# yzGuu830/efficient-speech-codec

Measured on AMD Instinct MI355X. Metric: audio-seconds/sec encode+decode, ESC-Base 9kbps 3s@16kHz, higher is better.
Workload: dtype f32 (fp32 storage and accumulation everywhere; the K = C contractions of the MLPs, of the attention's Q / K / V projections, of PatchMerge / PatchSplit and of the de-embedding run on the fp16 matrix cores with every fp32 operand split into two fp16 terms under power-of-two scales (range-safe by cons

## Files before the change

efficient-speech-codec_amd/csrc/escx_api.cpp:

```cpp
#include <hip/hip_runtime.h>

#include <algorithm>
#include <cmath>
#include <cstdlib>
#include <cstring>
#include <map>
#include <mutex>
#include <tuple>
#include <utility>
#include <vector>

#include "escx_internal.h"
#include "launchers.h"

using namespace escx;

static void part_layout(escx_handle_s* h, int B, int T, int* k, int* per, int* pass) {
    *k = std::min(n_parts(h, B), h->n_sets);
    *pass = std::max(1, std::min(pass_clips(h, B, T), h->sets[0].shp.B));
    *per = *k <= 1 ? B : (B + *k - 1) / *k;
}

template <class F>
static int run_halves(escx_handle_s* h, int B, int T, hipStream_t st, F part) {
// ... 179 lines not shown
             ln_rows(2, cur, h->xn, L.sub_g, L.sub_b, map, H2 * W, tokens, B * H2 * W, L.C, L.Cp, st));
        PROF("merge_gemm", 2.0 * B * H2 * W * 2 * L.C * L.Cout, (double)B * H2 * W * (2 * L.C + L.Cout) * 4,
             gemm_store(h->xn, 2 * L.Cp, B * H2 * W, L.sub_w, L.CoutP, 2 * L.Cp, y, L.CoutP, nullptr, st));
        }
        *Hout = H2;
    } else if (L.scale == 2) {
        int src2 = -1;
        if (h->use_fused)
            PROF("split_fused" + (h->prof ? "[C=" + std::to_string(L.C) + "]" : std::string()), 2.0 * M * L.C * 2 * L.Cout, (double)M * (L.C + 2 * L.Cout) * 4,
                 src2 = rowgemm_fused(1, cur, y, L.sub_g, L.sub_b, L.sub_wf, nullptr, M, tokens, tokens, L.C, L.Cp, 2 * L.CoutP, 1, H, W, L.CoutP, st, L.sub_x3, x3_nt(h)));
        if (src2 != 0) {
        PROF("split_ln", 0, 2.0 * M * L.C * 4,
             ln_rows(0, cur, h->xn, L.sub_g, L.sub_b, nullptr, tokens, tokens, M, L.C, L.Cp, st));
        PROF("split_gemm", 2.0 * M * L.C * 2 * L.Cout, (double)M * (L.C + 2 * L.Cout) * 4,
             gemm_split(h->xn, L.Cp, M, L.sub_w, 2 * L.CoutP, L.Cp, y, H, W, L.CoutP, st));
        }
        *Hout = 2 * H;
    } else {
        *Hout = H;
    }
    return launch_ok(L.prefix.c_str());
}

static int run_stft(escx_handle_s* h, const float* wave, int B, int L, int T, float* spec, hipStream_t st) {
    PROF("stft_dft_gemm", 2.0 * B * T * h->cfg.win_length * 2 * h->F, ((double)B * L + (double)B * T * 2 * h->F) * 4,
         gemm_frames(wave, B, L, T, h->cfg.hop_length, h->left - h->n_fft / 2, h->dft_w, h->cfg.in_dim * h->Fp, h->winP, spec, st));
    return launch_ok("stft");
}

static int run_patch_embed(escx_handle_s* h, const float* spec, int B, int T, int W, float* tok, hipStream_t st) {
    const escx_config& c = h->cfg;
    const int H0 = c.in_freq / c.patch_f;
    const double toks = (double)B * H0 * W;
    PROF("patch_embed_gemm", 2.0 * toks * c.in_dim * c.patch_f * c.patch_t * h->C0, ((double)B * T * 2 * h->F + toks * h->C0) * 4,
         gemm_patch(spec, B, T, c.in_dim, h->Fp, H0, W, c.patch_f, c.patch_t, h->pe_w, h->C0p, h->Kpe, tok, h->pe_b, st));
    PROF("patch_embed_ln", 0, 2 * toks * h->C0 * 4,
         ln_rows(0, tok, tok, h->pe_g, h->pe_beta, nullptr, H0 * W, H0 * W, B * H0 * W, h->C0, h->C0p, st));
    return launch_ok("patch_embed");
}

static int run_encoder(escx_handle_s* h, const Shapes& s, hipStream_t st) {
    int rc, H = s.H0, Hn;
    if ((rc = run_patch_embed(h, h->spec, s.B, s.T, s.W, h->stageA, st))) return rc;
    if ((rc = run_layer(h, h->layers[0], h->stageA, h->enc_hs[0], s.B, H, s.W, &Hn, st))) return rc;
    for (int i = 0; i + 1 < h->n; ++i) {
        if ((rc = run_layer(h, h->layers[1 + i], h->enc_hs[i], h->enc_hs[i + 1], s.B, H, s.W, &Hn, st))) return rc;
        H = Hn;
    }
    return 0;
}

static int ensure_pvq_tables(escx_handle_s* h, hipStream_t st) {
    if (!h->pvq_tab_stale) return 0;
    const escx_config& c = h->cfg;
    const int G = c.group_size, Ksz = c.codebook_size;
    const bool on = h->pvq_table;
    auto grab = [&](void** buf, size_t bytes) -> bool { return *buf || hipMalloc(buf, bytes) == hipSuccess; };
    if (on && !h->iota_codes) {
        std::vector<long long> iota((size_t)G * Ksz);
        for (int g = 0; g < G; ++g) for (int k = 0; k < Ksz; ++k) iota[(size_t)g * Ksz + k] = k;
        ESCX_HIP(hipMalloc((void**)&h->iota_codes, iota.size() * sizeof(long long)));
        ESCX_HIP(hipMemcpy(h->iota_codes, iota.data(), iota.size() * sizeof(long long), hipMemcpyHostToDevice));
    }
    for (Quant& q : h->quants) {
        if (!on || !q.tab_ok) { if (q.tab) { ESCX_HIP(hipDeviceSynchronize()); (void)hipFree(q.tab); q.tab = nullptr; } continue; }
        if (!q.tab) ESCX_HIP(hipMalloc((void**)&q.tab, (size_t)Ksz * q.Kq * sizeof(float)));
// ... 53 lines not shown
    const int Tq = W / c.overlap, M = B * Tq;
    const int splits = pvq_down_splits(M, q.Kq, q.Cp);
    if ((size_t)splits * M * q.Nz > h->zpart_cap) ESCX_FAIL(ESCX_ERR_STATE, "split-K scratch too small");
    const double vec = (double)c.overlap * q.Hq * q.C;
    PROF("pvq_down_gemm", 2.0 * M * vec * q.d, (double)M * vec * (dec ? 2 : 1) * 4,
         gemm_pvq_down(enc, dec, B, q.Hq, W, q.Cp, c.overlap, q.wd, q.Nz, q.Kq, h->zpart, splits, st));
    int src_rc = 0;
    PROF("pvq_search", 2.0 * M * c.group_size * c.codebook_size * q.d, ((double)c.group_size * c.codebook_size * q.d + (double)M * c.group_size * q.d) * 4,
         src_rc = pvq_search(h->zpart, splits, M, q.Nz, q.cbn, q.c2, q.cbraw, c.group_size, c.codebook_size, q.d, q.dt, Tq, codes, bstride,
                             loss, 1.0f / ((float)Tq * q.d * c.group_size), c.l2norm, st));
    if (src_rc) ESCX_FAIL(ESCX_ERR_UNSUPPORTED, "codebook_dim %d unsupported by the search kernel", q.d);
    return launch_ok("pvq_encode");
}

static int run_pvq_decode(escx_handle_s* h, const Quant& q, const long long* codes, long long bstride, const float* dec, int B, int W,
                          float* out, hipStream_t st) {
    const escx_config& c = h->cfg;
    const double vec = (double)c.overlap * q.Hq * q.C, Mv = (double)B * (W / c.overlap);
    const bool special = h->pvq_up_kernel;
    if (q.tab && special) {
        PROF("pvq_tab_add", 0, Mv * vec * (dec ? 3 : 2) * 4,
             pvq_tab_add(codes, bstride, q.tab, q.gq, c.group_size, c.codebook_size, B, q.Hq, W, q.Cp, c.overlap, dec, out, st));
        return launch_ok("pvq_decode");
    }
    int urc = -1;
    if (special)
        PROF("pvq_up_gemm", 2.0 * Mv * vec * q.d, Mv * vec * (dec ? 2 : 1) * 4,
             urc = pvq_up(codes, bstride, q.cbraw, c.group_size, c.codebook_size, q.dt, B, q.Hq, W, q.Cp, c.overlap, q.wup, q.Kq, q.Kup, dec, out, st));
    if (urc != 0) {
        if (special && h->prof && !h->prof_recs.empty()) h->prof_recs.pop_back();
    PROF("pvq_up_gemm", 2.0 * Mv * vec * q.d, Mv * vec * (dec ? 2 : 1) * 4,
         gemm_pvq_up(codes, bstride, q.cbraw, c.group_size, c.codebook_size, q.dt, B, q.Hq, W, q.Cp, c.overlap, q.wup, q.Kq, q.Kup, dec, out, st));
    }
    return launch_ok("pvq_decode");
}

static int run_pvq_quantize(escx_handle_s* h, const Quant& q, const float* enc, const float* dec, int B, int W, long long* codes, long long bstride,
                            float* loss, float* out, hipStream_t st) {
    const escx_config& c = h->cfg;
    if (h->pvq_fused) {
        const int Tq = W / c.overlap, M = B * Tq;
        const double vec = (double)c.overlap * q.Hq * q.C;
        int frc = -1;
        PROF(out ? "pvq_fused" : "pvq_fused_codes", 2.0 * M * vec * q.d * (out ? 2 : 1) + 2.0 * M * c.group_size * c.codebook_size * q.d,
             (double)M * vec * ((dec ? 2 : 1) + (out ? (dec ? 2 : 1) : 0)) * 4,
             frc = pvq_fused(enc, dec, B, q.Hq, W, q.Cp, c.overlap, q.wdf, q.Nz, q.Kq, pvq_down_splits(M, q.Kq, q.Cp), pvq_down_bk(q.Cp), q.cbn, q.c2, q.cbraw,
                             c.group_size, c.codebook_size, q.d, q.dt, q.wup, q.tab, q.gq, out, codes, bstride, loss, 1.0f / ((float)Tq * q.d * c.group_size), c.l2norm, st));
        if (frc == 0) return launch_ok("pvq_quantize");
        if (h->prof && !h->prof_recs.empty()) h->prof_recs.pop_back();
    }
    int rc;
    if ((rc = run_pvq_encode(h, q, enc, dec, B, W, codes, bstride, loss, st))) return rc;
    if (out && (rc = run_pvq_decode(h, q, codes, bstride, dec, B, W, out, st))) return rc;
    return 0;
}

static int run_deembed(escx_handle_s* h, const float* tok, int B, int W, float* rspec, hipStream_t st) {
    const escx_config& c = h->cfg;
    const int H0 = c.in_freq / c.patch_f;
    if (!h->deembed_two_stage && c.in_dim * h->Q <= 16) {
        const double tk = (double)B * H0 * W;
        int hrc = -1;
        if (h->deembed_halo)
            PROF("deembed_composed7x7", 2.0 * tk * 49 * h->C0 * c.in_dim * h->Q, (tk * h->C0 + tk * c.in_dim * h->Q) * 4,
                 hrc = deembed7_fused(tok, B, H0, W, h->C0p, h->dch_w, h->dcc_b, rspec, c.patch_f, c.patch_t, c.in_dim, h->Fp, st, h->dch_x2));
        if (hrc != 0)
// ... 52 lines not shown
        if ((rc = run_layer(h, h->layers[n + i], dec, other, s.B, H, s.W, &Hn, st))) return rc;
        std::swap(dec, other); H = Hn;
    }
    return 0;
}

extern "C" int escx_encode(escx_handle h, const float* wave, int B, int L, int S, int64_t* codes, int* fh, int* fw, void* stream) {
    if (h && h->kind == 1) return rvq_encode(h, wave, B, L, nullptr, S, codes, fh, fw, stream);
    int rc = check_ready(h); if (rc) return rc;
    if (!wave || !codes) ESCX_FAIL(ESCX_ERR_INVALID_ARG, "null pointer");
    if (S < 1 || S > h->cfg.max_streams) ESCX_FAIL(ESCX_ERR_INVALID_ARG, "num_streams=%d outside [1, %d]", S, h->cfg.max_streams);
    if (L <= h->n_fft / 2) ESCX_FAIL(ESCX_ERR_INVALID_ARG, "n_samples=%d too short for reflect padding of %d", L, h->n_fft / 2);
    Shapes s; if ((rc = ensure_ws(h, B, frames_of(h, L), &s))) return rc;
    const long long cstride = (long long)S * h->cfg.group_size * s.Tq;
    if ((rc = ensure_pvq_tables(h, (hipStream_t)stream))) return rc;
    rc = run_halves(h, B, s.T, (hipStream_t)stream, [&](int b0, int nb, hipStream_t st) -> int {
        Shapes sp = s; sp.B = nb; int r;
        if ((r = run_stft(h, wave + (size_t)b0 * L, nb, L, sp.T, h->spec, st))) return r;
        if ((r = run_encoder(h, sp, st))) return r;
        return run_csvq_encode(h, sp, S, (long long*)codes + b0 * cstride, st);
    });
    if (rc) return rc;
    if (fh) *fh = s.encH[h->n - 1];
    if (fw) *fw = s.W;
    return ESCX_OK;
}

static int run_csvq_decode(escx_handle_s* h, const long long* codes, int B, int S, int Hb, int W, float* rspec, hipStream_t st) {
    const escx_config& c = h->cfg;
    const int n = h->n, G = c.group_size, Tq = W / c.overlap;
    const long long bstride = (long long)S * G * Tq, sstride = (long long)G * Tq;
    int rc, H = Hb, Hn;
    float* dec = h->decA; float* other = h->decB;
    if ((rc = run_pvq_decode(h, h->quants[0], codes, bstride, nullptr, B, W, dec, st))) return rc;
    for (int i = 0; i + 1 < n; ++i) {
        if (i < S - 1 && (rc = run_pvq_decode(h, h->quants[i + 1], codes + (i + 1) * sstride, bstride, dec, B, W, dec, st))) return rc;
        if ((rc = run_layer(h, h->layers[n + i], dec, other, B, H, W, &Hn, st))) return rc;
        std::swap(dec, other); H = Hn;
    }
    if ((rc = run_layer(h, h->layers[2 * n - 1], dec, other, B, H, W, &Hn, st))) return rc;
    return run_deembed(h, other, B, W, rspec, st);
}

extern "C" int escx_decode(escx_handle h, const int64_t* codes, int B, int S, int fh, int fw, float* wave_out, float* recon_feat,
                           void* stream) {
    if (h && h->kind == 1) return rvq_decode(h, codes, B, S, nullptr, fh, fw, wave_out, recon_feat, stream);
    int rc = check_infer_ready(h); if (rc) return rc;
    if (!codes || !wave_out) ESCX_FAIL(ESCX_ERR_INVALID_ARG, "null pointer");
    const escx_config& c = h->cfg;
    if (S < 1 || S > c.max_streams) ESCX_FAIL(ESCX_ERR_INVALID_ARG, "codes.size(1)=%d outside [1, %d]", S, c.max_streams);
    if (fw < 1 || fw % c.overlap) ESCX_FAIL(ESCX_ERR_ASSERT, "Time dimension must be multiple of overlap");
    Shapes s; if ((rc = ensure_ws(h, B, frames_for_width(h, fw), &s))) return rc;
    if (s.W != fw || s.encH[h->n - 1] != fh) ESCX_FAIL(ESCX_ERR_INVALID_ARG, "feat_shape (%d,%d) does not match the model (%d,%d)", fh, fw, s.encH[h->n - 1], s.W);
    const int T2 = c.patch_t * fw, out_len = c.hop_length * (T2 - 1);
    const long long cstride = (long long)S * c.group_size * (fw / c.overlap);
    if ((rc = ensure_pvq_tables(h, (hipStream_t)stream))) return rc;
    rc = run_halves(h, B, s.T, (hipStream_t)stream, [&](int b0, int nb, hipStream_t st) -> int {
        int r;
        if ((r = run_csvq_decode(h, (const long long*)codes + b0 * cstride, nb, S, fh, fw, h->rspec, st))) return r;
        if ((r = run_istft(h, h->rspec, nb, T2, wave_out + (size_t)b0 * out_len, st))) return r;
        if (recon_feat) spec_unpad(h, h->rspec, recon_feat + (size_t)b0 * T2 * c.in_dim * h->F, (long long)nb * T2, st);
        return launch_ok("decode");
    });
    return rc;
}

static int forward_impl(escx_handle h, const float* wave, const float* feat, int B, int L, int T, int S, int64_t* codes, float* wave_out,
                        float* raw_feat, float* recon_feat, float* cm_loss, void* stream) {
    if (h && h->kind == 1) return rvq_forward(h, wave, feat, B, wave ? L : T, nullptr, S, codes, wave_out, raw_feat, recon_feat, cm_loss, stream);
// ... 119 lines not shown
    return 0;
}

static int upload_plan(escx_handle_s* h, const MixPlan& p, int32_t* dev, hipStream_t st) {
    ESCX_HIP(hipMemcpyAsync(dev, p.ints.data(), p.ints.size() * sizeof(int32_t), hipMemcpyHostToDevice, st));
    return 0;
}

static int clips_over(const int* S, int B, int j) { int c = 0; while (c < B && S[c] > j) ++c; return c; }

static int run_csvq_encode_streams(escx_handle_s* h, const Shapes& s, const int* S, long long* codes, long long bstride, hipStream_t st) {
    const int n = h->n;
    const long long sstride = (long long)h->cfg.group_size * s.Tq;
    int rc, H = s.encH[n - 1], Hn;
    float* dec = h->decA; float* other = h->decB;
    int nref = clips_over(S, s.B, 1);
    if ((rc = run_pvq_quantize(h, h->quants[0], h->enc_hs[n - 1], nullptr, s.B, s.W, codes, bstride, nullptr, nref ? dec : nullptr, st))) return rc;
    for (int i = 0; nref > 0; ++i) {
        const int nq = nref;
        nref = clips_over(S, nq, i + 2);
        if ((rc = run_pvq_quantize(h, h->quants[i + 1], h->enc_hs[n - 1 - i], dec, nq, s.W, codes + (i + 1) * sstride, bstride, nullptr, nref ? dec : nullptr, st))) return rc;
        if (!nref) break;
        if ((rc = run_layer(h, h->layers[n + i], dec, other, nref, H, s.W, &Hn, st))) return rc;
        std::swap(dec, other); H = Hn;
    }
    return 0;
}

static int run_csvq_decode_streams(escx_handle_s* h, const long long* codes, long long bstride, int B, const int* S, int Hb, int W, float* rspec, hipStream_t st) {
    const int n = h->n;
    const long long sstride = (long long)h->cfg.group_size * (W / h->cfg.overlap);
    int rc, H = Hb, Hn;
    float* dec = h->decA; float* other = h->decB;
    if ((rc = run_pvq_decode(h, h->quants[0], codes, bstride, nullptr, B, W, dec, st))) return rc;
    for (int i = 0; i + 1 < n; ++i) {
        const int nq = clips_over(S, B, i + 1);
        if (nq && (rc = run_pvq_decode(h, h->quants[i + 1], codes + (i + 1) * sstride, bstride, dec, nq, W, dec, st))) return rc;
        if ((rc = run_layer(h, h->layers[n + i], dec, other, B, H, W, &Hn, st))) return rc;
        std::swap(dec, other); H = Hn;
    }
    if ((rc = run_layer(h, h->layers[2 * n - 1], dec, other, B, H, W, &Hn, st))) return rc;
    return run_deembed(h, other, B, W, rspec, st);
}

extern "C" int escx_encode_streams(escx_handle h, const float* wave, int B, int L, const int32_t* streams, int64_t* codes, int* fh, int* fw,
                                   void* stream) {
    if (h && h->kind == 1) return rvq_encode(h, wave, B, L, streams, 0, codes, fh, fw, stream);
    int rc = check_ready(h); if (rc) return rc;
    if (!wave || !codes) ESCX_FAIL(ESCX_ERR_INVALID_ARG, "null pointer");
    int Smax = 0; if ((rc = check_streams(h, B, streams, &Smax))) return rc;
    if (L <= h->n_fft / 2) ESCX_FAIL(ESCX_ERR_INVALID_ARG, "n_samples=%d too short for reflect padding of %d", L, h->n_fft / 2);
    Shapes s; if ((rc = ensure_ws(h, B, frames_of(h, L), &s))) return rc;
    MixPlan p; plan_streams(h, B, s.T, streams, Smax, &p);
    const int GT = h->cfg.group_size * s.Tq;
    const long long cstride = (long long)Smax * GT;
    int32_t* maps; float* wave_ws; long long* codes_ws;
    MixBufs mb; mb.add(&maps, p.ints.size()); mb.add(&wave_ws, (size_t)B * L); mb.add(&codes_ws, (size_t)B * cstride);
    if ((rc = mix_alloc(h, mb))) return rc;
    hipStream_t st = (hipStream_t)stream;
    if ((rc = ensure_pvq_tables(h, st))) return rc;
    if ((rc = upload_plan(h, p, maps, st))) return rc;
    PROF("mix_gather", 0, 2.0 * B * L * 4, rows_permute(wave, wave_ws, maps, B, L, st));
    rc = run_halves(h, B, s.T, st, [&](int b0, int nb, hipStream_t sti) -> int {
        Shapes sp = s; sp.B = nb; int r;
        if ((r = run_stft(h, wave_ws + (size_t)b0 * L, nb, L, sp.T, h->spec, sti))) return r;
        if ((r = run_encoder(h, sp, sti))) return r;
        return run_csvq_encode_streams(h, sp, p.S_ws() + b0, codes_ws + b0 * cstride, cstride, sti);
    });
    if (rc) return rc;
// ... 450 lines not shown
```

efficient-speech-codec_amd/csrc/escx_internal.h:

```cpp
#pragma once
#include <hip/hip_runtime.h>
#include <cstdarg>
#include <cstdint>
#include <cstdio>
#include <map>
#include <string>
#include <tuple>
#include <vector>

#include "../../include/escx.h"

namespace escx {

inline int rup(int x, int m) { return (x + m - 1) / m * m; }

void set_error(const char* fmt, ...);

#define ESCX_FAIL(code, ...) do { ::escx::set_error(__VA_ARGS__); return (code); } while (0)
#define ESCX_HIP(expr) do { hipError_t _e = (expr); if (_e != hipSuccess) { \
        ::escx::set_error("%s failed: %s (%s:%d)", #expr, hipGetErrorString(_e), __FILE__, __LINE__); return ESCX_ERR_HIP; } } while (0)

struct Param { std::vector<float> data; std::vector<int64_t> shape; };

struct Arena {
// ... 66 lines not shown
namespace escx {
int make_shapes(escx_handle_s* h, int B, int T, Shapes* out);
int check_infer_ready(escx_handle_s* h);
void free_train_state(escx_handle_s* h);
int get_map(escx_handle_s* h, int H, int W, int shift, const int** out);
int check_ready(escx_handle_s* h);
float* stream_scratch(hipStream_t st, int slot, size_t floats);
int launch_ok(const char* what);
int build_gather_map(escx_handle_s* h);
void use_set(escx_handle_s* h, int i);
int n_parts(escx_handle_s* h, int B);
int ensure_ws(escx_handle_s* h, int B, int T, Shapes* s, int min_set_clips = 0);
int pass_clips(escx_handle_s* h, int B, int T);
}

struct escx_handle_s : escx::WsFields {
    escx_config cfg;
    int kind = 0;
    int num_rvqs = 0;
    int device = 0;
    int n = 0;
    int F = 0, Fp = 0, n_fft = 0, left = 0, winP = 0, Kpe = 0, C0 = 0, C0p = 0, Q = 0;
    std::map<std::string, escx::Param> params;
    std::vector<std::string> required;
    bool finalized = false;
    bool use_fused = true;
    bool use_fused_attn = true;
    int prec = 2;
    int mlp_x3_max = 384, attn_x3_max = 384;
    bool rowgemm_x3 = true, pvq_table = true;
    int attn_gs_tokens = 600;
    bool mlp_split_fold = true;
    bool pvq_fused = true, pvq_up_kernel = true;
    bool prof_serial = false;
    int ws = 4;

    escx::Arena wts;
    std::vector<escx::Layer> layers;
    std::vector<escx::Quant> quants;
    float *pe_w = nullptr, *pe_b = nullptr, *pe_g = nullptr, *pe_beta = nullptr;
    float *dc1_w = nullptr, *dc1_b = nullptr, *dc2_w = nullptr, *dc2_b = nullptr;
    float *dft_w = nullptr, *idft_w = nullptr, *win2 = nullptr;
    float *dcc_w = nullptr, *dcc_b = nullptr, *dcv_w = nullptr, *dcv_b = nullptr;
    float* dch_w = nullptr;
    void* dch_x2 = nullptr;
    void* dch_x2_buf = nullptr;
    float *dc1_wT = nullptr, *idft_wT = nullptr;
    float* dft_wT = nullptr;

    std::vector<std::string> flat_keys;
    std::vector<size_t> flat_off, flat_numel;
    size_t flat_total = 0;
    int* gmap = nullptr;
    float* garena = nullptr;
    std::vector<std::pair<size_t, size_t>> grad_regions;
    long long* grad_seg = nullptr; int grad_nseg = 0; long long grad_seg_total = 0;
    escx::Arena tape;
    void* train_state = nullptr;
    bool train_x3_stale = true;
    bool pvq_tab_stale = true;
    long long* iota_codes = nullptr;
    bool composed_stale = false;
    bool deembed_halo = true;
    bool deembed_two_stage = false;

    static constexpr int MAX_PARTS = 4;
// ... 43 lines not shown
```

efficient-speech-codec_amd/csrc/escx_params.cpp:

```cpp
#include <hip/hip_runtime.h>

#include <algorithm>
#include <cmath>
#include <cstdlib>
#include <cstring>
#include <map>
#include <mutex>
#include <tuple>

#include "escx_internal.h"
#include "launchers.h"

using namespace escx;

namespace escx {
static thread_local std::string g_err;
void set_error(const char* fmt, ...) {
    char buf[1024];
    va_list ap; va_start(ap, fmt); vsnprintf(buf, sizeof(buf), fmt, ap); va_end(ap);
    g_err = buf;
}
}

extern "C" const char* escx_last_error(void) { return g_err.c_str(); }
// ... 101 lines not shown
            K.push_back(p + "up_projs." + std::to_string(g) + ".weight");
        }
    for (const char* k : {"proj.weight", "proj.bias", "norm.weight", "norm.bias"}) K.push_back(std::string("encoder.patch_embed.") + k);
    for (const Layer& L : h->layers) {
        for (int j = 0; j < c.swin_depth; ++j) add_block_keys(K, L.prefix + "swint_blocks." + std::to_string(j) + ".");
        if (L.scale) {
            K.push_back(L.prefix + "subsample.norm.weight"); K.push_back(L.prefix + "subsample.norm.bias");
            K.push_back(L.prefix + (L.scale == 1 ? "subsample.down.weight" : "subsample.up.weight"));
        }
    }
    for (const char* k : {"de_proj1.weight", "de_proj1.bias", "de_proj2.weight", "de_proj2.bias"})
        K.push_back(std::string("decoder.patch_deembed.") + k);
    return 0;
}

static int env_defaults(escx_handle_s* h) {
    auto flag = [](const char* name, bool dflt) { const char* e = getenv(name); return (e && e[0]) ? e[0] == '1' : dflt; };
    auto off = [](const char* name) { const char* e = getenv(name); return e && e[0] == '0'; };
    auto num = [](const char* name, int dflt) { const char* e = getenv(name); return (e && e[0]) ? atoi(e) : dflt; };
    h->use_fused = !flag("ESCX_NO_FUSED", false);
    h->use_fused_attn = !flag("ESCX_NO_FUSED_ATTN", false);
    h->deembed_two_stage = flag("ESCX_DEEMBED_TWO_STAGE", false);
    h->deembed_halo = !flag("ESCX_DEEMBED_GEMM", false);
    if (getenv("ESCX_STREAMS") && getenv("ESCX_STREAMS")[0]) { h->parts = std::min(std::max(num("ESCX_STREAMS", 2), 1), (int)escx_handle_s::MAX_PARTS); h->parts_forced = true; }
    h->chunk_frames = num("ESCX_CHUNK_FRAMES", h->chunk_frames);
    h->mlp_x3_max = num("ESCX_MLP_X3", h->mlp_x3_max);
    h->attn_x3_max = num("ESCX_ATTN_X3", h->attn_x3_max);
    h->rowgemm_x3 = !off("ESCX_ROWGEMM_X3");
    h->pvq_table = !off("ESCX_PVQ_TABLE");
    h->attn_gs_tokens = num("ESCX_ATTN_GS_TOKENS", h->attn_gs_tokens);
    h->mlp_split_fold = !off("ESCX_MLP_SPLIT_FOLD");
    h->pvq_fused = !off("ESCX_PVQ_FUSED");
    h->pvq_up_kernel = !off("ESCX_PVQ_UP_KERNEL");
    h->prof_serial = flag("ESCX_PROF_SERIAL", false);
    if (num("ESCX_X3_TERMS", 2) == 3) h->prec = 3;
    if (const char* e = getenv("ESCX_PRECISION")) {
        if (e[0]) {
            const std::string v(e);
            if (v == "fp32" || v == "0") h->prec = 0; else if (v == "bf16x3" || v == "3") h->prec = 3; else if (v == "f16x2" || v == "2") h->prec = 2;
            else ESCX_FAIL(ESCX_ERR_INVALID_ARG, "ESCX_PRECISION=%s (fp32 | bf16x3 | f16x2)", e);
        }
    }
    return 0;
}

static int create_impl(const escx_config* cfg, int kind, int num_rvqs, int device, escx_handle* out) {
    int ndev = 0;
    ESCX_HIP(hipGetDeviceCount(&ndev));
    if (device < 0 || device >= ndev) ESCX_FAIL(ESCX_ERR_INVALID_ARG, "device %d out of range (%d visible)", device, ndev);
    escx_handle_s* h = new escx_handle_s();
    h->cfg = *cfg; h->device = device;
    h->kind = kind; h->num_rvqs = num_rvqs;
    int erc = env_defaults(h);
    if (erc) { delete h; return erc; }
    int rc = build_geometry(h);
    if (rc) { delete h; return rc; }
    *out = h;
    return ESCX_OK;
}

extern "C" int escx_create(const escx_config* cfg, int device, escx_handle* out) {
    if (!cfg || !out) ESCX_FAIL(ESCX_ERR_INVALID_ARG, "null argument");
    return create_impl(cfg, 0, 0, device, out);
}

extern "C" int escx_create_rvq(const escx_rvq_config* cfg, int device, escx_handle* out) {
// ... 744 lines not shown
```

efficient-speech-codec_amd/csrc/fused_pvq.h:

```cpp
#pragma once
#include <hip/hip_runtime.h>
#include "gemm_engine.h"
#include "kernels.h"

namespace escx {

struct PvqFusedArgs {
    const float* enc; const float* dec;
    const float* wd;
    const float* cbn; const float* c2; const float* cbraw;
    const float* wup;
    const float* tab; const float* gq;
    float* out;
    long long* codes; long long bstride;
    float* loss; float loss_scale;
    int M, Tq, Hq, Wd, Cp, ov, Kq, k_per_z, splits;
    int G, Ksz, d, l2norm;
    unsigned long long* trace;
};

constexpr int PVQF_WAVES = 16;
constexpr int PVQF_GMAX = 4;
template <int NT> constexpr int pvqf_lds_floats() { return PVQF_WAVES * 16 * (16 * NT + 4); }

// ... 249 lines not shown
                    for (int r = 0; r < 4; ++r) acc = __builtin_amdgcn_mfma_f32_16x16x4f32(wf[u][c][r], zf[c][r], acc, 0, 0, 0);
                if constexpr (DEC) acc += dv[u];
                if (live && nt0 + u < NTo) st4(a.out + idx[u], acc);
            }
        }
    }
    PVQ_TS(5)
#undef PVQ_TS
}

struct PvqTabAddArgs {
    const long long* codes; long long bstride; const float* tab; const float* gq; const float* dec; float* out;
    int G, Ksz, Tq, Hq, Wd, Cp, ov; long long n4;
};
__global__ __launch_bounds__(256) void pvq_tab_add_kernel(PvqTabAddArgs a) {
    ESCX_SET_PRIO_SMALL();
    const long long i = (long long)blockIdx.x * 256 + threadIdx.x;
    if (i >= a.n4) return;
    const int c4 = a.Cp >> 2;
    const long long row = i / c4; const int c = (int)(i - row * c4) * 4;
    const int w = (int)(row % a.Wd); const long long bh = row / a.Wd; const int h = (int)(bh % a.Hq); const int b = (int)(bh / a.Hq);
    const int t = w / a.ov, o = w - t * a.ov;
    const int g = (int)a.gq[(((o * a.Hq + h) * a.Cp) + c) >> 2];
    f32x4 v = zero4();
    if (g >= 0) {
        long long code = a.codes[(size_t)b * a.bstride + (size_t)g * a.Tq + t];
        code = code < 0 ? 0 : (code >= a.Ksz ? a.Ksz - 1 : code);
        v = ld4(a.tab + ((size_t)h * a.ov * a.Ksz + (size_t)a.ov * code + o) * a.Cp + c);
    }
    if (a.dec) v += ld4(a.dec + i * 4);
    st4(a.out + i * 4, v);
}

}
```

efficient-speech-codec_amd/csrc/gemm_engine.h:

```cpp
#pragma once
#include <hip/hip_runtime.h>
#include <cstdlib>
#include <type_traits>

#include "launch_prof.h"

#ifdef ESCX_SMALL_PRIO
#define ESCX_SET_PRIO_SMALL() __builtin_amdgcn_s_setprio(ESCX_SMALL_PRIO)
#else
#define ESCX_SET_PRIO_SMALL()
#endif

namespace escx {

typedef float f32x4 __attribute__((ext_vector_type(4)));

__device__ __forceinline__ f32x4 ld4(const float* p) { return *reinterpret_cast<const f32x4*>(p); }
__device__ __forceinline__ void st4(float* p, f32x4 v) { *reinterpret_cast<f32x4*>(p) = v; }
__device__ __forceinline__ f32x4 zero4() { f32x4 z = {0.f, 0.f, 0.f, 0.f}; return z; }

template <class E, class = void> struct epi_is_rowwise : std::false_type {};
template <class E> struct epi_is_rowwise<E, std::enable_if_t<E::ROWWISE>> : std::true_type {};

template <int BM, int BN, int BK, class Loader, class Epi>
// ... 270 lines not shown
    r = fmaf(r, u, -4.556713975034654e-05f);
    r = fmaf(r, u, 0.0005925663863308728f);
    r = fmaf(r, u, -0.004739245865494013f);
    r = fmaf(r, u, 0.026361873373389244f);
    r = fmaf(r, u, -0.10997311770915985f);
    r = fmaf(r, u, -0.6319426894187927f);
    r = fmaf(r, u, -1.130163311958313f);
    r = fmaf(r, u, 0.00030238047474995255f);
    const float b = copysignf(1.0f - exp_fast(r), x);
    return t <= 0.92f ? a : b;
}
__device__ __forceinline__ float gelu_bf(float x) {
    const float a = fabsf(x);
    float r = -1.6904631365832756e-06f;
    r = fmaf(r, a, 2.5084045773837715e-05f);
    r = fmaf(r, a, -0.0001144662601291202f);
    r = fmaf(r, a, -0.0003233331080991775f);
    r = fmaf(r, a, 0.007333371322602034f);
    r = fmaf(r, a, -0.052714187651872635f);
    r = fmaf(r, a, -0.4591154456138611f);
    r = fmaf(r, a, -1.151123285293579f);
    r = fmaf(r, a, 1.126017423302983e-06f - 1.0f);
    return fmaf(-fabsf(x), __builtin_amdgcn_exp2f(r), fmaxf(x, 0.0f));
}

struct EpiStore {
    float* out; int ldo; const float* bias;
    __device__ __forceinline__ void store(int m, int n, f32x4 v, int) const {
        if (bias) v += ld4(bias + n);
        st4(out + (size_t)m * ldo + n, v);
    }
};

struct EpiGelu {
    float* out; int ldo; const float* bias;
    __device__ __forceinline__ void store(int m, int n, f32x4 v, int) const {
        v += ld4(bias + n);
        v[0] = gelu_erf(v[0]); v[1] = gelu_erf(v[1]); v[2] = gelu_erf(v[2]); v[3] = gelu_erf(v[3]);
        st4(out + (size_t)m * ldo + n, v);
    }
};

struct EpiResidual {
    float* out; int ldo; const float* bias; const float* res;
    __device__ __forceinline__ void store(int m, int n, f32x4 v, int) const {
        v += ld4(bias + n);
        st4(out + (size_t)m * ldo + n, ld4(res + (size_t)m * ldo + n) + v);
    }
};

struct EpiQkv {
    float* out; int ldo; const float* bias; int nq; float scale;
    __device__ __forceinline__ void store(int m, int n, f32x4 v, int) const {
        v += ld4(bias + n);
        if (n < nq) v *= scale;
        st4(out + (size_t)m * ldo + n, v);
    }
};

struct EpiProjScatter {
    float* out; const float* shortcut; const float* bias; const int* map; int slots, tokens, Cp;
    __device__ __forceinline__ void store(int m, int n, f32x4 v, int) const {
        const int b = m / slots, s = m - b * slots;
        const int tok = map[s];
        if (tok < 0) return;
        const size_t idx = ((size_t)b * tokens + tok) * Cp + n;
// ... 115 lines not shown
```

efficient-speech-codec_amd/csrc/gemm_misc.hip:

```cpp
#include "gemm_engine.h"
#include "launchers.h"

namespace escx {

void gemm_frames(const float* wave, int B, int L, int T, int hop, int off, const float* W, int Np, int Kp, float* out, hipStream_t s) {
    FrameA ld{wave, L, T, hop, off, B * T, FastDiv(T)};
    launch_gemm<64>(ld, W, B * T, Np, Kp, EpiStore{out, Np, nullptr}, s);
}

void gemm_patch(const float* spec, int B, int T, int in_dim, int Fp, int H, int Wd, int pf, int pt, const float* W, int Np, int Kp,
                float* out, const float* bias, hipStream_t s) {
    PatchA ld{spec, T, in_dim * Fp, Fp, H, Wd, pf, pt, in_dim * pf * pt, B * H * Wd};
    launch_gemm<64>(ld, W, B * H * Wd, Np, Kp, EpiStore{out, Np, bias}, s);
}

void gemm_conv_deembed1(const float* x, int B, int H, int Wd, int Cp, const float* W, int Np, float* out, const float* bias, int pf,
                        int pt, hipStream_t s) {
    ConvA ld{x, H, Wd, Cp, 5, 5, B * H * Wd};
    const int M = B * H * Wd;
    if (M >= 32768) launch_gemm<128>(ld, W, M, Np, 25 * Cp, EpiDeembed1{out, bias, H, Wd, Cp, pf, pt}, s, 1, pick_bk(Cp));
    else launch_gemm<64>(ld, W, M, Np, 25 * Cp, EpiDeembed1{out, bias, H, Wd, Cp, pf, pt}, s, 1, pick_bk(Cp));
}

void gemm_conv_spec(const float* x, int B, int T, int F, int Cp, const float* W, float* out, const float* bias, int Fp, int in_dim,
                    hipStream_t s) {
    ConvA ld{x, T, F, Cp, 3, 3, B * T * F};
    launch_gemm<64>(ld, W, B * T * F, 16, 9 * Cp, EpiSpec{out, bias, T, F, Fp, in_dim}, s, 1, pick_bk(Cp));
}

int test_fastdiv(int n, int d) { return FastDiv(d).div(n); }

void gemm_deembed_composed(const float* x, int B, int H, int Wd, int Cp, const float* W, float* out, const float* bias, int pf, int pt,
                           int in_dim, int Fp, hipStream_t s) {
    ConvA ld{x, H, Wd, Cp, 7, 7, B * H * Wd};
    const int M = B * H * Wd;
    EpiDeembedC ep{out, bias, H, Wd, pf, pt, in_dim, Fp};
    if (M >= 32768) launch_gemm<128>(ld, W, M, 16, 49 * Cp, ep, s, 1, pick_bk(Cp));
    else launch_gemm<64>(ld, W, M, 16, 49 * Cp, ep, s, 1, pick_bk(Cp));
}

int pvq_down_splits(int , int Kp, int Cp) {
    const int BK = pick_bk(Cp);
    const int kIters = Kp / BK;
    int splits = kIters / 2;
    if (splits > 16) splits = 16;
    if (splits < 1) splits = 1;
// ... 22 lines not shown
```

efficient-speech-codec_amd/csrc/kernels_misc.hip:

```cpp
#include <algorithm>
#include <cstdint>

#include "kernels.h"
#include "fused_pvq.h"
#include "fused_prvq.h"
#include <atomic>
#include "launchers.h"

namespace escx {

static inline int grid_for(long long work_items, int per_block, int cap = 4096) {
    long long g = (work_items + per_block - 1) / per_block;
    if (g < 1) g = 1;
    if (g > cap) g = cap;
    return (int)g;
}

void ln_rows(int mode, const float* src, float* dst, const float* gamma, const float* beta, const int* map, int rows_per_clip,
             int src_rows_per_clip, int total_rows, int C, int Cp, hipStream_t s) {
    const int grid = grid_for(total_rows, 16, 8192);
    const float eps = 1e-5f;
    if (mode == 0)
        ESCX_LAUNCH((ln_rows_kernel<1, 0>), dim3(grid), dim3(256), 0, s, src, dst, gamma, beta, map, rows_per_clip,
                           src_rows_per_clip, total_rows, C, Cp, eps);
// ... 37 lines not shown
        default: return -1;
    }
#undef ESCX_SRCH
}

void loss_reduce(const float* terms, int n_slots, int G, int M, int Tq, float* out, hipStream_t s) {
    ESCX_LAUNCH(loss_reduce_kernel, dim3(M / Tq), dim3(64), 0, s, terms, n_slots, G, M, Tq, out);
}

template <int NT, int STEPS, bool DEC>
static void launch_pvq_fused_d(const PvqFusedArgs& a, hipStream_t s) {
    auto kern = pvq_fused_kernel<NT, STEPS, DEC>;
    constexpr int lds = pvqf_lds_floats<NT>() * (int)sizeof(float);
    if constexpr (lds > 48 * 1024) {
        static std::atomic<unsigned> done{0};
        int dev = 0; (void)hipGetDevice(&dev);
        const unsigned bit = 1u << (dev & 31);
        if (!(done.load(std::memory_order_relaxed) & bit)) {
            (void)hipFuncSetAttribute((const void*)kern, hipFuncAttributeMaxDynamicSharedMemorySize, lds);
            done.fetch_or(bit, std::memory_order_relaxed);
        }
    }
    ESCX_LAUNCH(kern, dim3((a.M + 15) / 16), dim3(64 * PVQF_WAVES), lds, s, a);
}
template <int NT, int STEPS>
static void launch_pvq_fused(const PvqFusedArgs& a, hipStream_t s) {
    if (a.dec) launch_pvq_fused_d<NT, STEPS, true>(a, s); else launch_pvq_fused_d<NT, STEPS, false>(a, s);
}

void pvq_tab_add(const long long* codes, long long bstride, const float* tab, const float* gq, int G, int Ksz, int B, int Hq, int Wd, int Cp, int ov,
                 const float* dec, float* out, hipStream_t s) {
    PvqTabAddArgs a{codes, bstride, tab, gq, dec, out, G, Ksz, Wd / ov, Hq, Wd, Cp, ov, (long long)B * Hq * Wd * (Cp / 4)};
    ESCX_LAUNCH(pvq_tab_add_kernel, dim3((unsigned)((a.n4 + 255) / 256)), dim3(256), 0, s, a);
}

int pvq_fused(const float* enc, const float* dec, int B, int Hq, int Wd, int Cp, int ov, const float* wd, int Np, int Kq, int splits, int bk,
              const float* cbn, const float* c2, const float* cbraw, int G, int Ksz, int d, int dt, const float* wup, const float* tab, const float* gq,
              float* out, long long* codes, long long bstride, float* loss, float loss_scale, int l2norm, hipStream_t s) {
    const int Tq = Wd / ov, M = B * Tq;
    if (Np % 16 || Kq % 16 || Cp % 16 || bk % 16 || Kq % bk || dt % 4 || G < 1 || G > PVQF_GMAX || G * dt > Np || splits < 1 || splits > PVQF_WAVES || Ksz < 1) return -1;
    const int kIters = Kq / bk, per = (kIters + splits - 1) / splits;
    if ((kIters + per - 1) / per != splits) return -1;
    PvqFusedArgs a{enc, dec, wd, cbn, c2, cbraw, wup, tab, gq, out, codes, bstride, loss, loss_scale, M, Tq, Hq, Wd, Cp, ov, Kq, per * bk, splits, G, Ksz, d, l2norm, nullptr};
#ifdef ESCX_PVQ_TRACE
    {
        static unsigned long long* last = nullptr; static int n = 0;
        unsigned long long* p = debug_trace_buffer();
        if (p != last) { last = p; n = 0; }
        a.trace = p ? p + (size_t)(n++ % 16) * 4096 * 8 : nullptr;
    }
#endif
    const int NT = Np / 16, STEPS = dt / 4;
    if (NT == 6 && STEPS == 8) { launch_pvq_fused<6, 8>(a, s); return 0; }
    if (NT == 3 && STEPS == 4) { launch_pvq_fused<3, 4>(a, s); return 0; }
    if (NT == 3 && STEPS == 3) { launch_pvq_fused<3, 3>(a, s); return 0; }
    if (NT == 2 && STEPS == 2) { launch_pvq_fused<2, 2>(a, s); return 0; }
    if (NT == 1 && STEPS == 1) { launch_pvq_fused<1, 1>(a, s); return 0; }
    return -1;
}

int pvq_up(const long long* codes, long long bstride, const float* cbraw, int G, int Ksz, int dt, int B, int Hq, int Wd, int Cp, int ov,
           const float* W, int Np, int Kp, const float* dec, float* out, hipStream_t s) {
    const int Tq = Wd / ov, M = B * Tq;
    if (Np % 16 || Kp % 16 || Cp % 16 || dt % 4) return -1;
    PvqUpArgs a{codes, bstride, cbraw, W, dec, out, G, Ksz, dt, Tq, M, Hq, Wd, Cp, ov, Kp, Np / 16, 0};
    const int mt = (M + 15) / 16;
// ... 133 lines not shown
```

efficient-speech-codec_amd/csrc/launchers.h:

```cpp
#pragma once
#include <hip/hip_runtime.h>

namespace escx {

void gemm_qkv(const float* A, int lda, int M, const float* W, int Np, int Kp, float* out, const float* bias,
              int nq, float scale, hipStream_t s);
void gemm_proj_scatter(const float* A, int lda, int M, const float* W, int Np, int Kp, float* out, const float* shortcut,
                       const float* bias, const int* map, int slots, int tokens, hipStream_t s);
void gemm_gelu(const float* A, int lda, int M, const float* W, int Np, int Kp, float* out, const float* bias, hipStream_t s);
void gemm_residual(const float* A, int lda, int M, const float* W, int Np, int Kp, float* out, const float* bias,
                   const float* res, hipStream_t s);
void gemm_store(const float* A, int lda, int M, const float* W, int Np, int Kp, float* out, int ldo, const float* bias, hipStream_t s);
void gemm_split(const float* A, int lda, int M, const float* W, int Np, int Kp, float* out, int H, int Wd, int C2p, hipStream_t s);

#ifndef ESCX_MLP_OCC4
#define ESCX_MLP_OCC4 96
#endif
#ifndef ESCX_ATTN_TMW2_MAX
#define ESCX_ATTN_TMW2_MAX 48
#endif
constexpr int attn_windows_per_wave(int Cp) { return Cp <= ESCX_ATTN_TMW2_MAX ? 2 : 1; }

constexpr int ESCX_COMB_UNSUPPORTED = -3;
struct MlpSplit { const float* wf; const float* gamma; const float* beta; float* out; int NT, H, W, C2p; };
// ... 6 lines not shown
int mlp_x3_pack(const float* w1, const float* w2, void* image, int Cp, int hiddenP, hipStream_t s, int nt = 3, const float* gamma = nullptr, const float* beta = nullptr,
                const float* b1 = nullptr, int C = 0);
struct MlpSplit;
int mlp_x3(float* x, int M, int C, int Cp, const float* gamma, const float* beta, const float* b1, const float* b2, const void* image, int hiddenP, int nw, int* hs_io, float* partial,
           hipStream_t s, const MlpSplit* split = nullptr, int nt = 3, float* out = nullptr);
size_t mlp_x3_split_bytes(int Cp, int Np);
int mlp_x3_split_pack(const float* wf, void* image, int Cp, int Np, hipStream_t s);
void rows_combine(float* dst, const float* src, const float* partial, const float* bias, long long M, int Cp, int n, hipStream_t s);

int rowgemm_fused(int segs, const float* x, float* out, const float* gamma, const float* beta, const float* wf, const int* map, int M,
                  int rows_per_clip, int src_rows_per_clip, int C, int Cp, int Np, int split, int H, int W, int C2p, hipStream_t s,
                  const void* x3_wf = nullptr, int x3_nt = 3);
size_t rowgemm_x3_bytes(int KP, int Np);
int rowgemm_x3_pack(const float* wf, void* image, int KP, int Np, hipStream_t s, int nt = 3, const float* gamma = nullptr, const float* beta = nullptr, int C = 0);
void loss_reduce(const float* terms, int n_slots, int G, int M, int Tq, float* out, hipStream_t s);
void mlp_set_trace(unsigned long long* p);
int test_fastdiv(int n, int d);
int deembed7_fused(const float* tok, int B, int H, int W, int Cp, const float* wfrag, const float* bias, float* out, int pf, int pt,
                   int in_dim, int Fp, hipStream_t s, const void* x2_image = nullptr);
size_t deembed7_x2_image_bytes(int Cp);
int deembed7_x2_pack(const float* wfrag, void* image, int Cp, hipStream_t s);
int attn_fused(const float* src, float* dst, int Cp, int C, int mode, int n_groups, const float* gamma, const float* beta,
               const float* wf, const float* bqkv, const float* bias_tab, const float* bproj, const int* map, int slots, int tokens,
               int n_windows, int nWh, int nWw, int shifted, float scale, int nw, int* gs_io, float* partial, int rows, hipStream_t s,
               const struct AttnTape* tape = nullptr,
               const void* x3_wf = nullptr, int x3_nt = 3);
size_t attn_x3_bytes(int Cp, int mode, int n_groups);
int attn_x3_pack(const float* waf, void* image, int Cp, int mode, int n_groups, hipStream_t s, int nt = 3, const float* gamma = nullptr, const float* beta = nullptr, int C = 0, const float* bqkv = nullptr);
struct AttnTape { float* xn; float* qkv; float* o; int ldq, ldo, hdp, nH; };

void gemm_frames(const float* wave, int B, int L, int T, int hop, int off, const float* W, int Np, int Kp, float* out, hipStream_t s);
void gemm_patch(const float* spec, int B, int T, int in_dim, int Fp, int H, int Wd, int pf, int pt, const float* W, int Np, int Kp,
                float* out, const float* bias, hipStream_t s);
void gemm_conv_deembed1(const float* x, int B, int H, int Wd, int Cp, const float* W, int Np, float* out, const float* bias,
                        int pf, int pt, hipStream_t s);
void gemm_conv_spec(const float* x, int B, int T, int F, int Cp, const float* W, float* out, const float* bias, int Fp, int in_dim,
                    hipStream_t s);
void gemm_deembed_composed(const float* x, int B, int H, int Wd, int Cp, const float* W, float* out, const float* bias, int pf, int pt,
                           int in_dim, int Fp, hipStream_t s);
int deembed_border(const float* x, const float* wv, const float* bv, float* out, int B, int H, int W, int C, int Cp, int pf, int pt,
                   int in_dim, int Fp, hipStream_t s);
void gemm_pvq_down(const float* enc, const float* dec, int B, int Hq, int Wd, int Cp, int ov, const float* W, int Np, int Kp,
                   float* zpart, int splits, hipStream_t s);
int pvq_down_splits(int M, int Kp, int Cp);
void gemm_pvq_up(const long long* codes, long long bstride, const float* cbraw, int G, int Ksz, int dt, int B, int Hq, int Wd, int Cp,
                 int ov, const float* W, int Np, int Kp, const float* dec, float* out, hipStream_t s);

void ln_rows(int mode, const float* src, float* dst, const float* gamma, const float* beta, const int* map, int rows_per_clip,
             int src_rows_per_clip, int total_rows, int C, int Cp, hipStream_t s);
int window_attention(const float* qkv, const float* bias, float* out, int total_windows, int nH, int hdp, int ldq, int ldo, int nWh,
                     int nWw, int shifted, hipStream_t s);
int window_attention_any(const float* qkv, const float* bias, float* out, int total_windows, int ws, int nH, int hd, int hdp, int ldq, int ldo, int nWh, int nWw,
                         int shift, hipStream_t s);
int pvq_fused(const float* enc, const float* dec, int B, int Hq, int Wd, int Cp, int ov, const float* wdf, int Np, int Kq, int splits, int bk,
              const float* cbn, const float* c2, const float* cbraw, int G, int Ksz, int d, int dt, const float* wup, const float* tab, const float* gq,
              float* out, long long* codes, long long bstride, float* loss, float loss_scale, int l2norm, hipStream_t s);
bool prvq_geometry_ok(int Np, int dt, int G, int Kq, int Cp, int splits, int bk);
int prvq_fused(const float* enc, const long long* codes_in, int B, int Hq, int Wd, int Cp, int ov, const float* wdf, int Np, int Kq, int splits, int bk,
               const float* cbn, const float* c2, const float* cbraw, int G, int Ksz, int d, int dt, const float* wup,
               long long* codes, long long bstride, const int* clip_S, int S, int Smax, float* loss, long long lslot, float loss_scale, int l2norm,
               float* out, hipStream_t s);
void pvq_tab_add(const long long* codes, long long bstride, const float* tab, const float* gq, int G, int Ksz, int B, int Hq, int Wd, int Cp, int ov,
                 const float* dec, float* out, hipStream_t s);
int pvq_down_bk(int Cp);
int pvq_up(const long long* codes, long long bstride, const float* cbraw, int G, int Ksz, int dt, int B, int Hq, int Wd, int Cp, int ov,
           const float* W, int Np, int Kp, const float* dec, float* out, hipStream_t s);
int pvq_search(const float* zpart, int splits, int M, int ldz, const float* cbn, const float* c2, const float* cbraw, int G, int Ksz,
               int d, int dt, int Tq, long long* codes, long long bstride, float* loss, float loss_scale, int l2norm, hipStream_t s);
void istft_ola(const float* frames, const float* win2, float* wave, int B, int T, int ldf, int win, int hop, int left, int half,
               int out_len, hipStream_t s);
void pad_rows(const float* src, float* dst, long long rows, int C, int Cp, hipStream_t s);
void unpad_rows(const float* src, float* dst, long long rows, int C, int Cp, hipStream_t s);
void codes_pack10(const long long* in, unsigned char* out, long long n, hipStream_t s);
void codes_unpack10(const unsigned char* in, long long* out, long long n, hipStream_t s);
void test_math(const float* x, float* y, long long n, int which, hipStream_t s);
void test_copy_rows(const float* src, float* dst, long long rows, int Cp, hipStream_t s);
void rows_permute(const float* src, float* dst, const int* map, int rows, long long row_len, hipStream_t s);
void codes_permute(const long long* src, long long src_stride, long long* dst, const int* map, const int* S, int rows, int Smax, int GT, hipStream_t s);
void loss_reduce_streams(const float* terms, long long lslot, const int* S, int cap, const int* slot_clips, int G, int Tq, int B, float* out, hipStream_t s);
void codes_pack10_streams(const long long* in, unsigned char* out, const long long* off, int B, long long clip_stride, long long n, hipStream_t s);
void codes_unpack10_streams(const unsigned char* in, long long* out, const long long* off, int B, long long clip_stride, hipStream_t s);
void codes_narrow(const long long* in, short* out, long long n, hipStream_t s);
void codes_widen(const short* in, long long* out, long long n, hipStream_t s);

}
```

Before: 11770.

## Fuse patch-embed LayerNorm into GEMM epilogue and merge first two PVQ table decodes

Adds a row-wise epilogue that stages the patch-embed GEMM tile in shared memory and applies bias plus LayerNorm before storing, replacing the separate LN pass. Also adds a kernel that gathers and sums the first two quantizer streams' codebook-table rows in one pass, replacing two pvq_tab_add launches and a read-modify-write of the decoder buffer. Both are gated by a new ESCX_FOLD_PASSES flag and fall back when shapes don't fit. The LN epilogue needs a tile spanning the whole padded row and extra shared memory, which could lower occupancy.

```diff
diff --git a/efficient-speech-codec_amd/csrc/escx_api.cpp b/efficient-speech-codec_amd/csrc/escx_api.cpp
--- a/efficient-speech-codec_amd/csrc/escx_api.cpp
+++ b/efficient-speech-codec_amd/csrc/escx_api.cpp
@@ -235,6 +235,13 @@
     const escx_config& c = h->cfg;
     const int H0 = c.in_freq / c.patch_f;
     const double toks = (double)B * H0 * W;
+    if (h->fold_passes) {
+        int frc = -1;
+        PROF("patch_embed_gemm", 2.0 * toks * c.in_dim * c.patch_f * c.patch_t * h->C0, ((double)B * T * 2 * h->F + toks * h->C0) * 4,
+             frc = gemm_patch_ln(spec, B, T, c.in_dim, h->Fp, H0, W, c.patch_f, c.patch_t, h->pe_w, h->C0p, h->Kpe, tok, h->pe_b, h->pe_g, h->pe_beta, h->C0, st));
+        if (frc == 0) return launch_ok("patch_embed");
+        if (h->prof && !h->prof_recs.empty()) h->prof_recs.pop_back();
+    }
     PROF("patch_embed_gemm", 2.0 * toks * c.in_dim * c.patch_f * c.patch_t * h->C0, ((double)B * T * 2 * h->F + toks * h->C0) * 4,
          gemm_patch(spec, B, T, c.in_dim, h->Fp, H0, W, c.patch_f, c.patch_t, h->pe_w, h->C0p, h->Kpe, tok, h->pe_b, st));
     PROF("patch_embed_ln", 0, 2 * toks * h->C0 * 4,
@@ -354,6 +361,20 @@
     PROF("pvq_up_gemm", 2.0 * Mv * vec * q.d, Mv * vec * (dec ? 2 : 1) * 4,
          gemm_pvq_up(codes, bstride, q.cbraw, c.group_size, c.codebook_size, q.dt, B, q.Hq, W, q.Cp, c.overlap, q.wup, q.Kq, q.Kup, dec, out, st));
     }
+    return launch_ok("pvq_decode");
+}
+
+static bool pvq_decode2_ok(const escx_handle_s* h) {
+    if (!h->fold_passes || !h->pvq_up_kernel || h->quants.size() < 2) return false;
+    const Quant& a = h->quants[0]; const Quant& b = h->quants[1];
+    return a.tab && b.tab && a.Hq == b.Hq && a.Cp == b.Cp && a.C == b.C;
+}
+static int run_pvq_decode2(escx_handle_s* h, const long long* codes0, const long long* codes1, long long bstride, int B, int W, float* out, hipStream_t st) {
+    const escx_config& c = h->cfg;
+    const Quant& q0 = h->quants[0]; const Quant& q1 = h->quants[1];
+    const double vec = (double)c.overlap * q0.Hq * q0.C, Mv = (double)B * (W / c.overlap);
+    PROF("pvq_tab_add", 0, Mv * vec * 3 * 4,
+         pvq_tab_add2(codes0, codes1, bstride, q0.tab, q0.gq, q1.tab, q1.gq, c.group_size, c.codebook_size, B, q0.Hq, W, q0.Cp, c.overlap, out, st));
     return launch_ok("pvq_decode");
 }
 
@@ -472,9 +493,12 @@
     const long long bstride = (long long)S * G * Tq, sstride = (long long)G * Tq;
     int rc, H = Hb, Hn;
     float* dec = h->decA; float* other = h->decB;
-    if ((rc = run_pvq_decode(h, h->quants[0], codes, bstride, nullptr, B, W, dec, st))) return rc;
+    const bool two = S >= 2 && n >= 2 && pvq_decode2_ok(h);
+    if (two) rc = run_pvq_decode2(h, codes, codes + sstride, bstride, B, W, dec, st);
+    else rc = run_pvq_decode(h, h->quants[0], codes, bstride, nullptr, B, W, dec, st);
+    if (rc) return rc;
     for (int i = 0; i + 1 < n; ++i) {
-        if (i < S - 1 && (rc = run_pvq_decode(h, h->quants[i + 1], codes + (i + 1) * sstride, bstride, dec, B, W, dec, st))) return rc;
+        if (i < S - 1 && !(two && i == 0) && (rc = run_pvq_decode(h, h->quants[i + 1], codes + (i + 1) * sstride, bstride, dec, B, W, dec, st))) return rc;
         if ((rc = run_layer(h, h->layers[n + i], dec, other, B, H, W, &Hn, st))) return rc;
         std::swap(dec, other); H = Hn;
     }
@@ -660,9 +684,12 @@
     const long long sstride = (long long)h->cfg.group_size * (W / h->cfg.overlap);
     int rc, H = Hb, Hn;
     float* dec = h->decA; float* other = h->decB;
-    if ((rc = run_pvq_decode(h, h->quants[0], codes, bstride, nullptr, B, W, dec, st))) return rc;
+    const bool two = n >= 2 && clips_over(S, B, 1) == B && pvq_decode2_ok(h);
+    if (two) rc = run_pvq_decode2(h, codes, codes + sstride, bstride, B, W, dec, st);
+    else rc = run_pvq_decode(h, h->quants[0], codes, bstride, nullptr, B, W, dec, st);
+    if (rc) return rc;
     for (int i = 0; i + 1 < n; ++i) {
-        const int nq = clips_over(S, B, i + 1);
+        const int nq = (two && i == 0) ? 0 : clips_over(S, B, i + 1);
         if (nq && (rc = run_pvq_decode(h, h->quants[i + 1], codes + (i + 1) * sstride, bstride, dec, nq, W, dec, st))) return rc;
         if ((rc = run_layer(h, h->layers[n + i], dec, other, B, H, W, &Hn, st))) return rc;
         std::swap(dec, other); H = Hn;
diff --git a/efficient-speech-codec_amd/csrc/escx_internal.h b/efficient-speech-codec_amd/csrc/escx_internal.h
--- a/efficient-speech-codec_amd/csrc/escx_internal.h
+++ b/efficient-speech-codec_amd/csrc/escx_internal.h
@@ -122,6 +122,7 @@
     int attn_gs_tokens = 600;
     bool mlp_split_fold = true;
     bool pvq_fused = true, pvq_up_kernel = true;
+    bool fold_passes = true;
     bool prof_serial = false;
     int ws = 4;
 
diff --git a/efficient-speech-codec_amd/csrc/escx_params.cpp b/efficient-speech-codec_amd/csrc/escx_params.cpp
--- a/efficient-speech-codec_amd/csrc/escx_params.cpp
+++ b/efficient-speech-codec_amd/csrc/escx_params.cpp
@@ -157,6 +157,7 @@
     h->mlp_split_fold = !off("ESCX_MLP_SPLIT_FOLD");
     h->pvq_fused = !off("ESCX_PVQ_FUSED");
     h->pvq_up_kernel = !off("ESCX_PVQ_UP_KERNEL");
+    h->fold_passes = !off("ESCX_FOLD_PASSES");
     h->prof_serial = flag("ESCX_PROF_SERIAL", false);
     if (num("ESCX_X3_TERMS", 2) == 3) h->prec = 3;
     if (const char* e = getenv("ESCX_PRECISION")) {
diff --git a/efficient-speech-codec_amd/csrc/fused_pvq.h b/efficient-speech-codec_amd/csrc/fused_pvq.h
--- a/efficient-speech-codec_amd/csrc/fused_pvq.h
+++ b/efficient-speech-codec_amd/csrc/fused_pvq.h
@@ -305,4 +305,32 @@
     st4(a.out + i * 4, v);
 }
 
+struct PvqTabAdd2Args {
+    const long long* codes0; const long long* codes1; long long bstride; const float* tab0; const float* gq0; const float* tab1; const float* gq1; float* out;
+    int G, Ksz, Tq, Hq, Wd, Cp, ov; long long n4;
+};
+__global__ __launch_bounds__(256) void pvq_tab_add2_kernel(PvqTabAdd2Args a) {
+    ESCX_SET_PRIO_SMALL();
+    const long long i = (long long)blockIdx.x * 256 + threadIdx.x;
+    if (i >= a.n4) return;
+    const int c4 = a.Cp >> 2;
+    const long long row = i / c4; const int c = (int)(i - row * c4) * 4;
+    const int w = (int)(row % a.Wd); const long long bh = row / a.Wd; const int h = (int)(bh % a.Hq); const int b = (int)(bh / a.Hq);
+    const int t = w / a.ov, o = w - t * a.ov;
+    const int gi = (((o * a.Hq + h) * a.Cp) + c) >> 2;
+    auto row_of = [&](const long long* codes, const float* tab, int g) {
+        f32x4 v = zero4();
+        if (g >= 0) {
+            long long code = codes[(size_t)b * a.bstride + (size_t)g * a.Tq + t];
+            code = code < 0 ? 0 : (code >= a.Ksz ? a.Ksz - 1 : code);
+            v = ld4(tab + ((size_t)h * a.ov * a.Ksz + (size_t)a.ov * code + o) * a.Cp + c);
+        }
+        return v;
+    };
+    const f32x4 v0 = row_of(a.codes0, a.tab0, (int)a.gq0[gi]);
+    f32x4 v1 = row_of(a.codes1, a.tab1, (int)a.gq1[gi]);
+    v1 += v0;
+    st4(a.out + i * 4, v1);
 }
+
+}
diff --git a/efficient-speech-codec_amd/csrc/gemm_engine.h b/efficient-speech-codec_amd/csrc/gemm_engine.h
--- a/efficient-speech-codec_amd/csrc/gemm_engine.h
+++ b/efficient-speech-codec_amd/csrc/gemm_engine.h
@@ -326,6 +326,62 @@
     }
 };
 
+template <int NP>
+struct EpiStoreLN {
+    static constexpr bool ROWWISE = true;
+    float* out; const float* bias; const float* gamma; const float* beta; int C; float eps;
+    __device__ __forceinline__ void store(int, int, f32x4, int) const {}
+    template <int TN, int TM>
+    __device__ __forceinline__ void finish(f32x4 (&acc)[TN][TM], int row0, int lane, int M) const {
+        static_assert(16 * TN == NP, "the workgroup tile spans exactly the padded row");
+        constexpr int LD = NP + 4, V = NP / 4, ROWS = 16 * TM;
+        __shared__ float stage[4 * ROWS * LD];
+        float* my = stage + (threadIdx.x >> 6) * ROWS * LD;
+        const int l15 = lane & 15, lg = lane >> 4;
+#pragma unroll
+        for (int b = 0; b < TM; ++b)
+#pragma unroll
+            for (int a = 0; a < TN; ++a) {
+                const int n = 16 * a + 4 * lg;
+                st4(my + (16 * b + l15) * LD + n, acc[a][b] + ld4(bias + n));
+            }
+        __syncthreads();
+        const int sub = lane & 15;
+        for (int r = lane >> 4; r < ROWS; r += 4) {
+            const int row = row0 + r;
+            if (row >= M) continue;
+            const float* sp = my + r * LD;
+            float* dp = out + (size_t)row * NP;
+            float sum = 0.f;
+            for (int v = sub; v < V; v += 16) {
+                f32x4 x = ld4(sp + 4 * v);
+#pragma unroll
+                for (int e = 0; e < 4; ++e) if (4 * v + e < C) sum += x[e];
+            }
+#pragma unroll
+            for (int o = 8; o >= 1; o >>= 1) sum += __shfl_xor(sum, o, 16);
+            const float mean = sum / (float)(C);
+            float var = 0.f;
+            for (int v = sub; v < V; v += 16) {
+                f32x4 x = ld4(sp + 4 * v);
+#pragma unroll
+                for (int e = 0; e < 4; ++e) if (4 * v + e < C) { const float d = x[e] - mean; var += d * d; }
+            }
+#pragma unroll
+            for (int o = 8; o >= 1; o >>= 1) var += __shfl_xor(var, o, 16);
+            const float rstd = 1.0f / sqrtf(var / (float)(C) + eps);
+            for (int v = sub; v < V; v += 16) {
+                f32x4 x = ld4(sp + 4 * v);
+                const f32x4 g = ld4(gamma + 4 * v), bb = ld4(beta + 4 * v);
+                f32x4 y;
+#pragma unroll
+                for (int e = 0; e < 4; ++e) y[e] = (4 * v + e < C) ? (x[e] - mean) * rstd * g[e] + bb[e] : 0.f;
+                st4(dp + 4 * v, y);
+            }
+        }
+    }
+};
+
 struct EpiGelu {
     float* out; int ldo; const float* bias;
     __device__ __forceinline__ void store(int m, int n, f32x4 v, int) const {
diff --git a/efficient-speech-codec_amd/csrc/gemm_misc.hip b/efficient-speech-codec_amd/csrc/gemm_misc.hip
--- a/efficient-speech-codec_amd/csrc/gemm_misc.hip
+++ b/efficient-speech-codec_amd/csrc/gemm_misc.hip
@@ -12,6 +12,29 @@
                 float* out, const float* bias, hipStream_t s) {
     PatchA ld{spec, T, in_dim * Fp, Fp, H, Wd, pf, pt, in_dim * pf * pt, B * H * Wd};
     launch_gemm<64>(ld, W, B * H * Wd, Np, Kp, EpiStore{out, Np, bias}, s);
+}
+
+template <int NP>
+static void launch_patch_ln(const PatchA& ld, const float* W, int M, int Kp, const EpiStoreLN<NP>& ep, hipStream_t s) {
+    switch (pick_bk(Kp)) {
+        case 80: launch_tile<64, NP, 80>(ld, W, M, NP, Kp, 1, ep, s); break;
+        case 48: launch_tile<64, NP, 48>(ld, W, M, NP, Kp, 1, ep, s); break;
+        case 32: launch_tile<64, NP, 32>(ld, W, M, NP, Kp, 1, ep, s); break;
+        default: launch_tile<64, NP, 16>(ld, W, M, NP, Kp, 1, ep, s); break;
+    }
+}
+
+int gemm_patch_ln(const float* spec, int B, int T, int in_dim, int Fp, int H, int Wd, int pf, int pt, const float* W, int Np, int Kp,
+                  float* out, const float* bias, const float* gamma, const float* beta, int C, hipStream_t s) {
+    if (!bias || pick_bn(Np) != Np) return -1;
+    PatchA ld{spec, T, in_dim * Fp, Fp, H, Wd, pf, pt, in_dim * pf * pt, B * H * Wd};
+    const int M = B * H * Wd;
+    const float eps = 1e-5f;
+    switch (Np) {
+        case 16: launch_patch_ln<16>(ld, W, M, Kp, EpiStoreLN<16>{out, bias, gamma, beta, C, eps}, s); return 0;
+        case 48: launch_patch_ln<48>(ld, W, M, Kp, EpiStoreLN<48>{out, bias, gamma, beta, C, eps}, s); return 0;
+        default: return -1;
+    }
 }
 
 void gemm_conv_deembed1(const float* x, int B, int H, int Wd, int Cp, const float* W, int Np, float* out, const float* bias, int pf,
diff --git a/efficient-speech-codec_amd/csrc/kernels_misc.hip b/efficient-speech-codec_amd/csrc/kernels_misc.hip
--- a/efficient-speech-codec_amd/csrc/kernels_misc.hip
+++ b/efficient-speech-codec_amd/csrc/kernels_misc.hip
@@ -93,6 +93,12 @@
                  const float* dec, float* out, hipStream_t s) {
     PvqTabAddArgs a{codes, bstride, tab, gq, dec, out, G, Ksz, Wd / ov, Hq, Wd, Cp, ov, (long long)B * Hq * Wd * (Cp / 4)};
     ESCX_LAUNCH(pvq_tab_add_kernel, dim3((unsigned)((a.n4 + 255) / 256)), dim3(256), 0, s, a);
+}
+
+void pvq_tab_add2(const long long* codes0, const long long* codes1, long long bstride, const float* tab0, const float* gq0, const float* tab1, const float* gq1,
+                  int G, int Ksz, int B, int Hq, int Wd, int Cp, int ov, float* out, hipStream_t s) {
+    PvqTabAdd2Args a{codes0, codes1, bstride, tab0, gq0, tab1, gq1, out, G, Ksz, Wd / ov, Hq, Wd, Cp, ov, (long long)B * Hq * Wd * (Cp / 4)};
+    ESCX_LAUNCH(pvq_tab_add2_kernel, dim3((unsigned)((a.n4 + 255) / 256)), dim3(256), 0, s, a);
 }
 
 int pvq_fused(const float* enc, const float* dec, int B, int Hq, int Wd, int Cp, int ov, const float* wd, int Np, int Kq, int splits, int bk,
diff --git a/efficient-speech-codec_amd/csrc/launchers.h b/efficient-speech-codec_amd/csrc/launchers.h
--- a/efficient-speech-codec_amd/csrc/launchers.h
+++ b/efficient-speech-codec_amd/csrc/launchers.h
@@ -62,6 +62,8 @@
 void gemm_frames(const float* wave, int B, int L, int T, int hop, int off, const float* W, int Np, int Kp, float* out, hipStream_t s);
 void gemm_patch(const float* spec, int B, int T, int in_dim, int Fp, int H, int Wd, int pf, int pt, const float* W, int Np, int Kp,
                 float* out, const float* bias, hipStream_t s);
+int gemm_patch_ln(const float* spec, int B, int T, int in_dim, int Fp, int H, int Wd, int pf, int pt, const float* W, int Np, int Kp,
+                  float* out, const float* bias, const float* gamma, const float* beta, int C, hipStream_t s);
 void gemm_conv_deembed1(const float* x, int B, int H, int Wd, int Cp, const float* W, int Np, float* out, const float* bias,
                         int pf, int pt, hipStream_t s);
 void gemm_conv_spec(const float* x, int B, int T, int F, int Cp, const float* W, float* out, const float* bias, int Fp, int in_dim,
@@ -92,6 +94,8 @@
                float* out, hipStream_t s);
 void pvq_tab_add(const long long* codes, long long bstride, const float* tab, const float* gq, int G, int Ksz, int B, int Hq, int Wd, int Cp, int ov,
                  const float* dec, float* out, hipStream_t s);
+void pvq_tab_add2(const long long* codes0, const long long* codes1, long long bstride, const float* tab0, const float* gq0, const float* tab1, const float* gq1,
+                  int G, int Ksz, int B, int Hq, int Wd, int Cp, int ov, float* out, hipStream_t s);
 int pvq_down_bk(int Cp);
 int pvq_up(const long long* codes, long long bstride, const float* cbraw, int G, int Ksz, int dt, int B, int Hq, int Wd, int Cp, int ov,
            const float* W, int Np, int Kp, const float* dec, float* out, hipStream_t s);
```

New measurement: 11760, median of 2. No clear change (-0.1%).
